# colinsongf/keyword_spotting

Hardware: AMD Instinct MI355X
Metric: mel-frames/s (real-time 10 ms-hop audio streams sustained = value/100) (higher is better)
Workload: dtype f32

## Files before the change

keyword_spotting_amd/csrc/gru_kernels.hip:

```cpp
#include <cstddef>

#include "gru_device.h"
#include "window_device.h"

namespace kws {

template <int KCX, bool FIRST, bool LAST, bool WINDOW = false>
__global__ void __launch_bounds__(256) __attribute__((amdgpu_waves_per_eu(1, 1)))
gru_layer_resident(const GruLayerParams p) {
    static_assert(!WINDOW || (LAST && !FIRST), "the window tail belongs to the last layer of a stack");
    constexpr int H = 128, NT = 8, KCH = 32;
    const int tid = threadIdx.x;
    const int w = __builtin_amdgcn_readfirstlane(tid >> 6);
    const int lane = tid & 63, g = lane >> 4, s = lane & 15;
    const int n_groups = (p.B + kStreamsPerGroup - 1) / kStreamsPerGroup;
    int group = blockIdx.x;
    int b_raw = group * kStreamsPerGroup + s;
    bool bvalid = b_raw < p.B;
    int b = bvalid ? b_raw : p.B - 1;
    const int T = p.T;
    const int n0 = 2 * w, n1 = 2 * w + 1;

    extern __shared__ __attribute__((aligned(16))) char smem[];
    f32x4* hbuf = reinterpret_cast<f32x4*>(smem);
    f32x4* rhbuf = hbuf + NT * 64;
    f32x4* wlds = rhbuf + NT * 64;
    EpilogueLds epi = epilogue_carve(reinterpret_cast<char*>(wlds + 4 * KCX * 64));
    if constexpr (WINDOW) epi.cwords = reinterpret_cast<int8_t*>(reinterpret_cast<char*>(wlds + 4 * KCX * 64) + kEpilogueLdsBytes);
    const uint8_t* win_dl = reinterpret_cast<const uint8_t*>(epi.cwords) + 16 * kWinTailWordsStride;
    constexpr size_t kWinOffset = offsetof(GruLayerParams, win);
    if constexpr (WINDOW) window_tail_prepare(window_tail_params_from_kernarg(kWinOffset), const_cast<uint8_t*>(win_dl), tid);
    constexpr int kXsStride = xs_stride(KCX);
    float* xs = reinterpret_cast<float*>(reinterpret_cast<char*>(wlds + 4 * KCX * 64) + (LAST ? kEpilogueLdsBytes : 0));

    float wgh[2][2][KCH];
    float wch[2][KCH];
    float wcx[2][KCX];
    const f32x4* wh4 = reinterpret_cast<const f32x4*>(p.wh);
#pragma unroll
    for (int j = 0; j < 2; ++j) {
        const int n = 2 * w + j;
#pragma unroll
        for (int k4 = 0; k4 < KCH / 4; ++k4) {
            const f32x4 vr = wh4[((n * 3 + 0) * (KCH / 4) + k4) * 64 + lane];
            const f32x4 vu = wh4[((n * 3 + 1) * (KCH / 4) + k4) * 64 + lane];
            const f32x4 vc = wh4[((n * 3 + 2) * (KCH / 4) + k4) * 64 + lane];
#pragma unroll
            for (int e = 0; e < 4; ++e) {
                wgh[j][0][4 * k4 + e] = vr[e];
                wgh[j][1][4 * k4 + e] = vu[e];
                wch[j][4 * k4 + e] = vc[e];
            }
        }
    }
    if constexpr (FIRST) {
#pragma unroll
        for (int j = 0; j < 2; ++j)
#pragma unroll
            for (int kc = 0; kc < KCX; ++kc) wcx[j][kc] = p.wx[(((2 * w + j) * 3 + 2) * KCX + kc) * 64 + lane];
        for (int kc = 0; kc < KCX; ++kc) {
            f32x4 v;
            v.x = p.wx[((n0 * 3 + 0) * KCX + kc) * 64 + lane];
            v.y = p.wx[((n0 * 3 + 1) * KCX + kc) * 64 + lane];
            v.z = p.wx[((n1 * 3 + 0) * KCX + kc) * 64 + lane];
            v.w = p.wx[((n1 * 3 + 1) * KCX + kc) * 64 + lane];
            wlds[(w * KCX + kc) * 64 + lane] = v;
        }
    } else {
        const f32x4* wx4 = reinterpret_cast<const f32x4*>(p.wx);
#pragma unroll
        for (int j = 0; j < 2; ++j)
#pragma unroll
            for (int k4 = 0; k4 < KCX / 4; ++k4) {
                const f32x4 vc = wx4[(((2 * w + j) * 3 + 2) * (KCX / 4) + k4) * 64 + lane];
#pragma unroll
                for (int e = 0; e < 4; ++e) wcx[j][4 * k4 + e] = vc[e];
            }
        for (int k4 = 0; k4 < KCX / 4; ++k4) {
            const f32x4 r0 = wx4[((n0 * 3 + 0) * (KCX / 4) + k4) * 64 + lane];
            const f32x4 u0 = wx4[((n0 * 3 + 1) * (KCX / 4) + k4) * 64 + lane];
            const f32x4 r1 = wx4[((n1 * 3 + 0) * (KCX / 4) + k4) * 64 + lane];
            const f32x4 u1 = wx4[((n1 * 3 + 1) * (KCX / 4) + k4) * 64 + lane];
#pragma unroll
            for (int e = 0; e < 4; ++e)
                wlds[(w * KCX + 4 * k4 + e) * 64 + lane] = (f32x4){r0[e], u0[e], r1[e], u1[e]};
        }
    }
#pragma unroll
    for (int j = 0; j < 2; ++j) {
#pragma unroll
        for (int kc = 0; kc < KCH; ++kc) {
            asm volatile("" : "+a"(wgh[j][0][kc]));
            asm volatile("" : "+a"(wgh[j][1][kc]));
            asm volatile("" : "+a"(wch[j][kc]));
        }
    }
    asm volatile("s_nop 7" ::: "memory");
    f32x4 bias_r[2], bias_u[2], bias_c[2];
#pragma unroll
    for (int j = 0; j < 2; ++j) {
        const int n = 2 * w + j;
        bias_r[j] = ld4(p.bias + 0 * H + n * 16 + 4 * g);
        bias_u[j] = ld4(p.bias + 1 * H + n * 16 + 4 * g);
        bias_c[j] = ld4(p.bias + 2 * H + n * 16 + 4 * g);
    }
    float wfc[2][4];
    f32x4 bfc4 = splat4(0.f);
    if (LAST) {
#pragma unroll
        for (int j = 0; j < 2; ++j)
#pragma unroll
            for (int e = 0; e < 4; ++e) wfc[j][e] = p.wfc[((2 * w + j) * 4 + e) * 64 + lane];
        if (w == 0) bfc4 = ld4(p.bfc + 4 * g);
    }

    int len_s = T;
    f32x4 hreg[2];
    const float4* xl_src = nullptr;
    const float4* xprev = nullptr;
    constexpr int XQ = KCX;
    const int xl_row = lane / XQ, xl_q = lane % XQ;
    const bool xl_active = FIRST && lane < 4 * XQ;
    auto enter_group = [&]() {
        b_raw = group * kStreamsPerGroup + s;
        bvalid = b_raw < p.B;
        b = bvalid ? b_raw : p.B - 1;
        const bool do_reset = p.reset != nullptr && p.reset[b] != 0;
        len_s = p.seq_len ? p.seq_len[b] - p.t_base : T;
#pragma unroll
        for (int j = 0; j < 2; ++j) {
            const int n = 2 * w + j;
            hreg[j] = do_reset ? splat4(0.f) : ld4(p.state_in + (size_t)b * H + n * 16 + 4 * g);
            hbuf[n * 64 + lane] = hreg[j];
        }
        if (LAST && tid < 16) {
            const int bb = group * kStreamsPerGroup + tid;
            int pw = -1;
            if (bb < p.B && p.prev_word && !(p.reset && p.reset[bb])) pw = p.prev_word[bb];
            epi.carry[tid] = pw;
        }
        if constexpr (FIRST) {
            const int xl_b = min(group * kStreamsPerGroup + 4 * w + (xl_active ? xl_row : 0), p.B - 1);
            xl_src = reinterpret_cast<const float4*>(p.x_mel + (size_t)xl_b * (p.t_stride ? p.t_stride : T) * p.I) + xl_q;
        } else {
            xprev = p.x_prev + (size_t)group * T * NT * 64 + lane;
        }
    };

    float4 xl_inflight = make_float4(0.f, 0.f, 0.f, 0.f);
    auto coop_issue = [&](int t_req) {
        const int t = t_req < T ? t_req : T - 1;
        if (xl_active) xl_inflight = xl_src[(size_t)t * XQ];
    };
    auto coop_commit = [&]() {
        if (xl_active) {
            float* dst = xs + (4 * (4 * w + xl_row)) * kXsStride + xl_q;
            dst[0 * kXsStride] = xl_inflight.x;
            dst[1 * kXsStride] = xl_inflight.y;
            dst[2 * kXsStride] = xl_inflight.z;
            dst[3 * kXsStride] = xl_inflight.w;
        }
    };
    float xbuf0[KCX];
    auto read_xs = [&](float (&dst)[KCX]) {
        const float* row = xs + (4 * s + g) * kXsStride;
#pragma unroll
        for (int k4 = 0; k4 < KCX / 4; ++k4) {
            const f32x4 v = *reinterpret_cast<const f32x4*>(row + 4 * k4);
            dst[4 * k4 + 0] = v[0]; dst[4 * k4 + 1] = v[1]; dst[4 * k4 + 2] = v[2]; dst[4 * k4 + 3] = v[3];
        }
        if constexpr (KCX % 4 >= 2) {
            const f32x2 v = *reinterpret_cast<const f32x2*>(row + (KCX / 4) * 4);
            dst[(KCX / 4) * 4 + 0] = v[0]; dst[(KCX / 4) * 4 + 1] = v[1];
        }
        if constexpr (KCX % 2 == 1) dst[KCX - 1] = row[KCX - 1];
    };
    auto load_x_slice = [&](float (&dst)[KCX], int t_req, const int sl) {
        if constexpr (!FIRST) {
            const int t = t_req < T ? t_req : T - 1;
            const float4 v = xprev[((size_t)t * NT + sl) * 64];
            dst[4 * sl + 0] = v.x; dst[4 * sl + 1] = v.y; dst[4 * sl + 2] = v.z; dst[4 * sl + 3] = v.w;
        }
    };

    f32x4 acc_r[2], acc_u[2], acc_c[2];
    auto gates_x_part = [&](const float (&xB)[KCX], auto k0_, auto k1_, auto pin_) {
        constexpr int K0 = decltype(k0_)::value, K1 = decltype(k1_)::value;
        constexpr bool PIN = decltype(pin_)::value;
        f32x4 ring[3];
        if (K0 < K1) ring[K0 % 3] = wlds[(w * KCX + K0) * 64 + lane];
        if (K0 + 1 < K1) ring[(K0 + 1) % 3] = wlds[(w * KCX + K0 + 1) * 64 + lane];
#pragma unroll
        for (int kc = K0; kc < K1; ++kc) {
            if (kc + 2 < K1) ring[(kc + 2) % 3] = wlds[(w * KCX + kc + 2) * 64 + lane];
            if (PIN) __builtin_amdgcn_sched_barrier(0);
            const f32x4 a4 = ring[kc % 3];
            acc_r[0] = mfma4(a4.x, xB[kc], acc_r[0]);
            acc_u[0] = mfma4(a4.y, xB[kc], acc_u[0]);
            acc_r[1] = mfma4(a4.z, xB[kc], acc_r[1]);
            acc_u[1] = mfma4(a4.w, xB[kc], acc_u[1]);
            if (PIN) __builtin_amdgcn_sched_barrier(0);
        }
    };
    using pinned = std::true_type;
    constexpr int KSPLIT = KCX / 2;
    using k_lo = std::integral_constant<int, 0>;
    using k_mid = std::integral_constant<int, KSPLIT>;
    using k_hi = std::integral_constant<int, KCX>;
    auto cand_x = [&](const float (&xB)[KCX]) {
#pragma unroll
        for (int j = 0; j < 2; ++j) acc_c[j] = bias_c[j];
#pragma unroll
        for (int kc = 0; kc < KCX; ++kc) {
            acc_c[0] = mfma4(wcx[0][kc], xB[kc], acc_c[0]);
            acc_c[1] = mfma4(wcx[1][kc], xB[kc], acc_c[1]);
        }
    };

    f32x4 hb_a, hb_b;

    auto frame = [&](int t, float (&xcur)[KCX], float (&xnxt)[KCX]) {
        mfma_prefence(acc_r[0], acc_u[0], acc_r[1], acc_u[1]);
#pragma unroll
        for (int nn = 0; nn < NT; ++nn) {
            const f32x4 hb = (nn & 1) ? hb_b : hb_a;
            if (nn + 2 < NT) {
                if (nn & 1) hb_b = hbuf[(nn + 2) * 64 + lane]; else hb_a = hbuf[(nn + 2) * 64 + lane];
            }
            if constexpr (FIRST) { if (nn == 0) coop_issue(t + 2); } else load_x_slice(xnxt, t + 1, nn);
            __builtin_amdgcn_sched_barrier(0);
#pragma unroll
            for (int e = 0; e < 4; ++e) {
                const int kc = 4 * nn + e;
                const float hv = hb[e];
                KWS_MFMA_A(acc_r[0], wgh[0][0][kc], hv);
                KWS_MFMA_A(acc_u[0], wgh[0][1][kc], hv);
                KWS_MFMA_A(acc_r[1], wgh[1][0][kc], hv);
                KWS_MFMA_A(acc_u[1], wgh[1][1][kc], hv);
            }
        }
        mfma_fence(acc_r[0], acc_u[0], acc_r[1], acc_u[1]);
        if constexpr (FIRST) read_xs(xcur);
        f32x4 u[2];
#pragma unroll
        for (int j = 0; j < 2; ++j) {
            const f32x2 r_lo = sigmoid2((f32x2){acc_r[j][0], acc_r[j][1]});
            const f32x2 r_hi = sigmoid2((f32x2){acc_r[j][2], acc_r[j][3]});
            const f32x2 rh_lo = r_lo * (f32x2){hreg[j][0], hreg[j][1]};
            const f32x2 rh_hi = r_hi * (f32x2){hreg[j][2], hreg[j][3]};
            rhbuf[(2 * w + j) * 64 + lane] = (f32x4){rh_lo.x, rh_lo.y, rh_hi.x, rh_hi.y};
        }
#pragma unroll
        for (int j = 0; j < 2; ++j) {
            const f32x2 u_lo = sigmoid2((f32x2){acc_u[j][0], acc_u[j][1]});
            const f32x2 u_hi = sigmoid2((f32x2){acc_u[j][2], acc_u[j][3]});
            u[j] = (f32x4){u_lo.x, u_lo.y, u_hi.x, u_hi.y};
        }
#pragma unroll
        for (int j = 0; j < 2; ++j) { acc_r[j] = bias_r[j]; acc_u[j] = bias_u[j]; }
        __builtin_amdgcn_sched_barrier(0);
        gates_x_part(xcur, k_lo{}, k_mid{}, pinned{});
        lds_barrier();
        hb_a = rhbuf[0 * 64 + lane];
        hb_b = rhbuf[1 * 64 + lane];
        gates_x_part(xcur, k_mid{}, k_hi{}, pinned{});

        mfma_prefence(acc_c[0], acc_c[1]);
#pragma unroll
        for (int nn = 0; nn < NT; ++nn) {
            const f32x4 rb = (nn & 1) ? hb_b : hb_a;
            if (nn + 2 < NT) {
                if (nn & 1) hb_b = rhbuf[(nn + 2) * 64 + lane]; else hb_a = rhbuf[(nn + 2) * 64 + lane];
            }
            __builtin_amdgcn_sched_barrier(0);
#pragma unroll
            for (int e = 0; e < 4; ++e) {
                const int kc = 4 * nn + e;
                const float rv = rb[e];
                KWS_MFMA_A(acc_c[0], wch[0][kc], rv);
                KWS_MFMA_A(acc_c[1], wch[1][kc], rv);
            }
        }
        mfma_fence(acc_c[0], acc_c[1]);
        const unsigned live = t < len_s ? 0xffffffffu : 0u;
        f32x4 hout[2];
#pragma unroll
        for (int j = 0; j < 2; ++j) {
#pragma unroll
            for (int h2 = 0; h2 < 2; ++h2) {
                const f32x2 c = tanh2((f32x2){acc_c[j][2 * h2], acc_c[j][2 * h2 + 1]});
                const f32x2 uu = {u[j][2 * h2], u[j][2 * h2 + 1]};
                const f32x2 hh = {hreg[j][2 * h2], hreg[j][2 * h2 + 1]};
                const f32x2 hn = (1.0f - uu) * c + uu * hh;
                hreg[j][2 * h2] = bitsel(live, hn.x, hh.x);
                hreg[j][2 * h2 + 1] = bitsel(live, hn.y, hh.y);
                if (LAST) {
                    hout[j][2 * h2] = bitsel(live, hn.x, 0.f);
                    hout[j][2 * h2 + 1] = bitsel(live, hn.y, 0.f);
                }
            }
        }
#pragma unroll
        for (int j = 0; j < 2; ++j) acc_c[j] = bias_c[j];
        constexpr int NCX = 2 * KCX;
        constexpr int NPOST = NCX >= 32 ? 16 : 8;
        constexpr int NPRE = NCX - NPOST;
        auto cand_x_mfma = [&](auto mc) {
            constexpr int m = decltype(mc)::value, kc = m / 2;
            if constexpr (m % 2 == 0) acc_c[0] = mfma4(wcx[0][kc], xcur[kc], acc_c[0]);
            else acc_c[1] = mfma4(wcx[1][kc], xcur[kc], acc_c[1]);
        };
        if constexpr (FIRST) coop_commit();
#pragma unroll
        for (int j = 0; j < 2; ++j) {
            hbuf[(2 * w + j) * 64 + lane] = hreg[j];
            if (!LAST) {
                const f32x4 o = hreg[j];
                p.h_out[((size_t)group * T + t) * NT * 64 + (2 * w + j) * 64 + lane] =
                    make_float4(o[0], o[1], o[2], o[3]);
            }
        }
        if (LAST) {
            f32x4 accf = bfc4;
#pragma unroll
            for (int j = 0; j < 2; ++j)
#pragma unroll
                for (int e = 0; e < 4; ++e) accf = mfma4(wfc[j][e], hout[j][e], accf);
            if (g < 2) *reinterpret_cast<f32x4*>(epi.pstage + (w * 16 + s) * 8 + 4 * g) = accf;
        }
        __builtin_amdgcn_sched_barrier(0);
        static_for<0, NPRE>(cand_x_mfma);
        __builtin_amdgcn_sched_barrier(0);
        lds_barrier();
        hb_a = hbuf[0 * 64 + lane];
        hb_b = hbuf[1 * 64 + lane];
        FoldRegs fold;
        const bool folder = LAST && w == (t & 3);
        if (folder) epilogue_fold_load(epi, lane, fold);
        __builtin_amdgcn_sched_barrier(0);
        static_for<NPRE, NCX>(cand_x_mfma);
        __builtin_amdgcn_sched_barrier(0);
        if (LAST) {
            if (folder) epilogue_fold_store(epi, t, lane, fold);
            if (((t + 1) & (kRingFrames - 1)) == 0 || t == T - 1) {
                const int t0 = t & ~(kRingFrames - 1);
                lds_barrier();
                epilogue_flush(p, epi, group, t0, t - t0 + 1, w, lane, t == T - 1);
            }
        }
    };

    for (; group < n_groups; group += gridDim.x) {
    enter_group();
    __syncthreads();
    if (T > 0) {
        if constexpr (FIRST) {
            coop_issue(0);
            coop_commit();
            __syncthreads();
            read_xs(xbuf0);
            coop_issue(1);
        } else {
#pragma unroll
            for (int sl = 0; sl < NT; ++sl) load_x_slice(xbuf0, 0, sl);
        }
#pragma unroll
        for (int j = 0; j < 2; ++j) { acc_r[j] = bias_r[j]; acc_u[j] = bias_u[j]; }
        gates_x_part(xbuf0, k_lo{}, k_hi{}, pinned{});
        hb_a = hbuf[0 * 64 + lane];
        hb_b = hbuf[1 * 64 + lane];
        cand_x(xbuf0);
        if constexpr (FIRST) {
            __syncthreads();
            coop_commit();
            __syncthreads();
        }
    }
    for (int t = 0; t < T; ++t) frame(t, xbuf0, xbuf0);

    if (bvalid) {
#pragma unroll
        for (int j = 0; j < 2; ++j)
            *reinterpret_cast<f32x4*>(p.state_out + (size_t)b * H + (2 * w + j) * 16 + 4 * g) = hreg[j];
    }
    __syncthreads();
    if constexpr (WINDOW) {
        const WindowTail win = window_tail_params_from_kernarg(kWinOffset);
        WindowTailRegs<2> wreq;
        window_tail_request<2>(win, p.B, group * kStreamsPerGroup, tid, wreq);
        window_tail<2>(win, p.B, group * kStreamsPerGroup, T, epi.cwords, kWinTailWordsStride, win_dl, reinterpret_cast<char*>(hbuf), tid, wreq);
        __syncthreads();
    }
    }
}

constexpr float kResidualScale = 0.7071067811865475f;
constexpr float kLayerNormEps = 1e-5f;

template <int TPW, bool FIRST, bool LAST, bool PIPE, bool WRAP = false>
__device__ __forceinline__ void gru_layer_generic_body(const GruLayerParams& p, const int group,
                                                       const GruWrapLayer& wl = GruWrapLayer{nullptr, 0.f, 0}) {
    constexpr int NT = 4 * TPW, H = 64 * TPW;
    const int tid = threadIdx.x;
    const int w = __builtin_amdgcn_readfirstlane(tid >> 6);
    const int lane = tid & 63, g = lane >> 4, s = lane & 15;
    const int b_raw = group * kStreamsPerGroup + s;
    const bool bvalid = b_raw < p.B;
    const int b = bvalid ? b_raw : p.B - 1;
    const int T = p.T, I = p.I;
    const int KCX4 = p.KCX / 4;

    extern __shared__ __attribute__((aligned(16))) char smem[];
    f32x4* hbuf = reinterpret_cast<f32x4*>(smem);
    f32x4* rhbuf = hbuf + NT * 64;
    f32x4* xstage = rhbuf + NT * 64;
    f32x4* biasl = xstage + NT * 64;
    const EpilogueLds epi = epilogue_carve(reinterpret_cast<char*>(biasl + 3 * NT * 4));
    f32x4* const xln = WRAP ? reinterpret_cast<f32x4*>(reinterpret_cast<char*>(biasl + 3 * NT * 4) + kEpilogueLdsBytes) : nullptr;
    const bool w_ln = WRAP && wl.igamma != nullptr;
    const bool w_res = WRAP && !FIRST && wl.residual != 0;
    const bool w_staged = w_ln || w_res;

    const __amdgpu_buffer_rsrc_t wx_rsrc = __builtin_amdgcn_make_buffer_rsrc(const_cast<float*>(p.wx), (short)0, 0x7fffffff, 0x00020000);
    const __amdgpu_buffer_rsrc_t wh_rsrc = __builtin_amdgcn_make_buffer_rsrc(const_cast<float*>(p.wh), (short)0, 0x7fffffff, 0x00020000);
    const int lane16 = lane * 16;
    auto bload = [&](const __amdgpu_buffer_rsrc_t& r, int frag) -> f32x4 {
        return __builtin_bit_cast(f32x4, __builtin_amdgcn_raw_buffer_load_b128(r, lane16, frag * 1024, 0));
    };

    f32x4 hreg[TPW];
    const bool do_reset = p.reset != nullptr && p.reset[b] != 0;
    const int len_s = p.seq_len ? p.seq_len[b] - p.t_base : T;
    for (int i = tid; i < 3 * NT * 4; i += 256) biasl[i] = ld4(p.bias + 4 * i);
#pragma unroll
    for (int j = 0; j < TPW; ++j) {
        const int n = TPW * w + j;
        hreg[j] = do_reset ? splat4(0.f) : ld4(p.state_in + (size_t)b * H + n * 16 + 4 * g);
        hbuf[n * 64 + lane] = hreg[j];
    }
    f32x4 bfc4 = splat4(0.f);
    if (LAST) {
        if (w == 0) bfc4 = ld4(p.bfc + 4 * g);
        if (tid < 16) {
            const int bb = group * kStreamsPerGroup + tid;
            int pw = -1;
            if (bb < p.B && p.prev_word && !(p.reset && p.reset[bb])) pw = p.prev_word[bb];
            epi.carry[tid] = pw;
        }
    }
    const float* xrow = FIRST ? p.x_mel + (size_t)b * (p.t_stride ? p.t_stride : T) * I : nullptr;
    const __amdgpu_buffer_rsrc_t xp_rsrc = __builtin_amdgcn_make_buffer_rsrc(
        FIRST ? const_cast<float*>(p.wh) : const_cast<float*>(reinterpret_cast<const float*>(p.x_prev + (size_t)group * T * NT * 64)),
        (short)0, 0x7fffffff, 0x00020000);
    const __amdgpu_buffer_rsrc_t ho_rsrc = __builtin_amdgcn_make_buffer_rsrc(
        LAST ? const_cast<float*>(p.wh) : reinterpret_cast<float*>(p.h_out + (size_t)group * T * NT * 64), (short)0, 0x7fffffff, 0x00020000);
    constexpr int kSysScope = 1 | 16;
    const bool vec_ok = (I & 3) == 0;
    __syncthreads();

    auto x_operand = [&](int t, int k4) -> f32x4 {
        f32x4 xb;
        if (WRAP && w_staged) {
            xb = (w_ln ? xln : xstage)[k4 * 64 + lane];
        } else if (FIRST) {
            const int k = 16 * k4 + 4 * g;
            const float* src = xrow + (size_t)t * I + k;
            if (vec_ok && k + 3 < I) {
                xb = ld4(src);
            } else {
#pragma unroll
                for (int e = 0; e < 4; ++e) xb[e] = (k + e < I) ? src[e] : 0.f;
            }
        } else if (PIPE) {
            xb = xstage[k4 * 64 + lane];
        } else {
            xb = bload(xp_rsrc, t * NT + k4);
        }
        return xb;
    };
    constexpr int RT = TPW, NP = TPW / RT;
    struct RowX { f32x4 a[RT][3]; f32x4 xb; };
    struct RowH { f32x4 a[RT][2]; };
    struct RowC { f32x4 a[RT]; };
    auto load_x = [&](RowX& r, int t, int q) {
        const int qq = q < KCX4 * NP ? q : KCX4 * NP - 1, kk = qq / NP, part = qq - kk * NP;
#pragma unroll
        for (int j = 0; j < RT; ++j)
#pragma unroll
            for (int c = 0; c < 3; ++c) r.a[j][c] = bload(wx_rsrc, ((TPW * w + part * RT + j) * 3 + c) * KCX4 + kk);
        r.xb = x_operand(t, kk);
        __builtin_amdgcn_sched_barrier(0);
    };
    auto load_h = [&](RowH& r, int q) {
        const int qq = q < NT * NP ? q : NT * NP - 1, kk = qq / NP, part = qq - kk * NP;
#pragma unroll
        for (int j = 0; j < RT; ++j)
#pragma unroll
            for (int c = 0; c < 2; ++c) r.a[j][c] = bload(wh_rsrc, ((TPW * w + part * RT + j) * 3 + c) * NT + kk);
        __builtin_amdgcn_sched_barrier(0);
    };
    auto load_c = [&](RowC& r, int q) {
        const int qq = q < NT * NP ? q : NT * NP - 1, kk = qq / NP, part = qq - kk * NP;
#pragma unroll
        for (int j = 0; j < RT; ++j) r.a[j] = bload(wh_rsrc, ((TPW * w + part * RT + j) * 3 + 2) * NT + kk);
        __builtin_amdgcn_sched_barrier(0);
    };
    auto mel_operand = [&](int t, int k4) -> f32x4 {
        f32x4 xb;
        const int k = 16 * k4 + 4 * g;
        const float* src = xrow + (size_t)t * I + k;
        if (vec_ok && k + 3 < I) {
            xb = ld4(src);
        } else {
#pragma unroll
            for (int e = 0; e < 4; ++e) xb[e] = (k + e < I) ? src[e] : 0.f;
        }
        return xb;
    };
    auto wrap_frame = [&](int t) {
        f32x4* const raw = FIRST ? xln : xstage;
        if (FIRST) {
            for (int k0 = w; k0 < KCX4; k0 += 16) {
                f32x4 v[4];
#pragma unroll
                for (int i = 0; i < 4; ++i) if (k0 + 4 * i < KCX4) v[i] = mel_operand(t, k0 + 4 * i);
#pragma unroll
                for (int i = 0; i < 4; ++i) if (k0 + 4 * i < KCX4) raw[(k0 + 4 * i) * 64 + lane] = v[i];
            }
            __syncthreads();
        } else if (!PIPE) {
            f32x4 v[NT / 4];
#pragma unroll
            for (int i = 0; i < NT / 4; ++i) v[i] = bload(xp_rsrc, t * NT + w + 4 * i);
#pragma unroll
            for (int i = 0; i < NT / 4; ++i) raw[(w + 4 * i) * 64 + lane] = v[i];
            __syncthreads();
        }
        if (!w_ln) return;
        float sum = 0.f;
        for (int k4 = 0; k4 < KCX4; ++k4) {
            const f32x4 v = raw[k4 * 64 + lane];
            sum += (v[0] + v[1]) + (v[2] + v[3]);
        }
        sum += __shfl_xor(sum, 16);
        sum += __shfl_xor(sum, 32);
        const float mu = sum / (float)I;
        float sq = 0.f;
        for (int k4 = 0; k4 < KCX4; ++k4) {
            const f32x4 v = raw[k4 * 64 + lane];
#pragma unroll
            for (int e = 0; e < 4; ++e) {
                float d = v[e] - mu;
                if (FIRST) d = (16 * k4 + 4 * g + e < I) ? d : 0.f;
                sq = fmaf(d, d, sq);
            }
        }
        sq += __shfl_xor(sq, 16);
        sq += __shfl_xor(sq, 32);
        const float scale = wl.ibeta * rsqrtf(sq / (float)I + kLayerNormEps);
        if (FIRST) __syncthreads();
        for (int k0 = w; k0 < KCX4; k0 += 16) {
            f32x4 gm[4];
#pragma unroll
            for (int i = 0; i < 4; ++i) if (k0 + 4 * i < KCX4) gm[i] = ld4(wl.igamma + 16 * (k0 + 4 * i) + 4 * g);
#pragma unroll
            for (int i = 0; i < 4; ++i) {
                const int k4 = k0 + 4 * i;
                if (k4 < KCX4) {
                    const f32x4 v = raw[k4 * 64 + lane];
                    f32x4 o;
#pragma unroll
                    for (int e = 0; e < 4; ++e) {
                        o[e] = fmaf(v[e] - mu, scale, gm[i][e]);
                        if (FIRST) o[e] = (16 * k4 + 4 * g + e < I) ? o[e] : 0.f;
                    }
                    xln[k4 * 64 + lane] = o;
                }
            }
        }
        __syncthreads();
    };
    for (int t = 0; t < T; ++t) {
        f32x4 acc_r[TPW], acc_u[TPW], acc_c[TPW];
#pragma unroll
        for (int j = 0; j < TPW; ++j) {
            const int n = TPW * w + j;
            acc_r[j] = biasl[(0 * NT + n) * 4 + g]; acc_u[j] = biasl[(1 * NT + n) * 4 + g]; acc_c[j] = biasl[(2 * NT + n) * 4 + g];
        }
        if (PIPE && !FIRST) {
            int spins = 0;
            while (__hip_atomic_load(p.ready_in + group, __ATOMIC_RELAXED, __HIP_MEMORY_SCOPE_AGENT) <= t) {
                __builtin_amdgcn_s_sleep(2);
                if (++spins > (1 << 24)) { if (lane == 0) *reinterpret_cast<volatile int*>(p.pipe_error) = 1; break; }
            }
            asm volatile("" ::: "memory");
            f32x4 xv[NT / 4];
#pragma unroll
            for (int i = 0; i < NT / 4; ++i)
                xv[i] = __builtin_bit_cast(f32x4, __builtin_amdgcn_raw_buffer_load_b128(xp_rsrc, lane16, (t * NT + (w + 4 * i)) * 1024, kSysScope));
#pragma unroll
            for (int i = 0; i < NT / 4; ++i) xstage[(w + 4 * i) * 64 + lane] = xv[i];
            __syncthreads();
        }
        if constexpr (WRAP) {
            if (w_staged) wrap_frame(t);
        }
        {
#define KWS_MMA_X(P_)                                                                                 \
            _Pragma("unroll") for (int j = 0; j < RT; ++j)                                             \
                _Pragma("unroll") for (int e = 0; e < 4; ++e) {                                        \
                    acc_r[P_ * RT + j] = mfma4(rr.a[j][0][e], rr.xb[e], acc_r[P_ * RT + j]);           \
                    acc_u[P_ * RT + j] = mfma4(rr.a[j][1][e], rr.xb[e], acc_u[P_ * RT + j]);           \
                    acc_c[P_ * RT + j] = mfma4(rr.a[j][2][e], rr.xb[e], acc_c[P_ * RT + j]);           \
                }
            RowX ra, rb;
            const int NQ = KCX4 * NP;
            load_x(ra, t, 0);
#pragma nounroll
            for (int q = 0; q < NQ; q += 2) {
                load_x(rb, t, q + 1);
                { const RowX& rr = ra; KWS_MMA_X(0); __builtin_amdgcn_sched_barrier(0); }
                if (q + 1 < NQ) {
                    load_x(ra, t, q + 2);
                    { const RowX& rr = rb; if (NP == 2) { KWS_MMA_X((NP - 1)); } else { KWS_MMA_X(0); } __builtin_amdgcn_sched_barrier(0); }
                }
            }
#undef KWS_MMA_X
        }
        {
#define KWS_MMA_H(P_)                                                                                 \
            _Pragma("unroll") for (int j = 0; j < RT; ++j)                                             \
                _Pragma("unroll") for (int e = 0; e < 4; ++e) {                                        \
                    acc_r[P_ * RT + j] = mfma4(rr.a[j][0][e], hb[e], acc_r[P_ * RT + j]);              \
                    acc_u[P_ * RT + j] = mfma4(rr.a[j][1][e], hb[e], acc_u[P_ * RT + j]);              \
                }
            RowH ra, rb;
            constexpr int NQ = NT * NP;
            load_h(ra, 0);
#pragma nounroll
            for (int q = 0; q < NQ; q += 2) {
                load_h(rb, q + 1);
                { const RowH& rr = ra; const f32x4 hb = hbuf[(q / NP) * 64 + lane]; KWS_MMA_H(0); __builtin_amdgcn_sched_barrier(0); }
                load_h(ra, q + 2);
                { const RowH& rr = rb; const f32x4 hb = hbuf[((q + 1) / NP) * 64 + lane];
                  if (NP == 2) { KWS_MMA_H((NP - 1)); } else { KWS_MMA_H(0); } __builtin_amdgcn_sched_barrier(0); }
            }
#undef KWS_MMA_H
        }
        f32x4 u[TPW];
#pragma unroll
        for (int j = 0; j < TPW; ++j) {
            f32x4 rh;
#pragma unroll
            for (int e = 0; e < 4; ++e) {
                rh[e] = sigmoid_f(acc_r[j][e]) * hreg[j][e];
                u[j][e] = sigmoid_f(acc_u[j][e]);
            }
            rhbuf[(TPW * w + j) * 64 + lane] = rh;
        }
        RowC ca, cb;
        if (PIPE && !LAST) asm volatile("s_waitcnt vmcnt(0)" ::: "memory");
        load_c(ca, 0);
        __syncthreads();
        if (PIPE && !LAST && t > 0 && tid == 0)
            __hip_atomic_store(p.ready_out + group, t, __ATOMIC_RELAXED, __HIP_MEMORY_SCOPE_AGENT);
        {
#define KWS_MMA_C(P_)                                                                                 \
            _Pragma("unroll") for (int j = 0; j < RT; ++j)                                             \
                _Pragma("unroll") for (int e = 0; e < 4; ++e)                                          \
                    acc_c[P_ * RT + j] = mfma4(rr.a[j][e], rb[e], acc_c[P_ * RT + j]);
            constexpr int NQ = NT * NP;
#pragma nounroll
            for (int q = 0; q < NQ; q += 2) {
                load_c(cb, q + 1);
                { const RowC& rr = ca; const f32x4 rb = rhbuf[(q / NP) * 64 + lane]; KWS_MMA_C(0); __builtin_amdgcn_sched_barrier(0); }
                load_c(ca, q + 2);
                { const RowC& rr = cb; const f32x4 rb = rhbuf[((q + 1) / NP) * 64 + lane];
                  if (NP == 2) { KWS_MMA_C((NP - 1)); } else { KWS_MMA_C(0); } __builtin_amdgcn_sched_barrier(0); }
            }
#undef KWS_MMA_C
        }
        const unsigned live = t < len_s ? 0xffffffffu : 0u;
        f32x4 accf = bfc4;
#pragma unroll
        for (int j = 0; j < TPW; ++j) {
            const int n = TPW * w + j;
            f32x4 hout;
            f32x4 xr = splat4(0.f), seam = splat4(0.f);
            if (WRAP && w_res) xr = xstage[n * 64 + lane];
#pragma unroll
            for (int e = 0; e < 4; ++e) {
                const float c = tanh_f(acc_c[j][e]);
                const float hn = fmaf(u[j][e], hreg[j][e], (1.0f - u[j][e]) * c);
                hreg[j][e] = bitsel(live, hn, hreg[j][e]);
                hout[e] = bitsel(live, hn, 0.f);
                if (WRAP) {
                    const float o = w_res ? kResidualScale * (hn + xr[e]) : hn;
                    hout[e] = bitsel(live, o, 0.f);
                    seam[e] = bitsel(live, o, hreg[j][e]);
                }
            }
            hbuf[n * 64 + lane] = hreg[j];
            if (!LAST) {
                const f32x4 o = WRAP ? seam : hreg[j];
                float4* dst = p.h_out + ((size_t)group * T + t) * NT * 64 + n * 64 + lane;
                if (PIPE) {
                    typedef int i32x4 __attribute__((ext_vector_type(4)));
                    __builtin_amdgcn_raw_buffer_store_b128(__builtin_bit_cast(i32x4, o), ho_rsrc, lane16, (t * NT + n) * 1024, kSysScope);
                } else {
                    *dst = make_float4(o[0], o[1], o[2], o[3]);
                }
            } else {
#pragma unroll
                for (int e = 0; e < 4; ++e) accf = mfma4(p.wfc[(n * 4 + e) * 64 + lane], hout[e], accf);
            }
        }
        if (LAST && g < 2) *reinterpret_cast<f32x4*>(epi.pstage + (w * 16 + s) * 8 + 4 * g) = accf;
        __syncthreads();
        if (LAST) {
            if (w == (t & 3)) epilogue_fold(epi, t, lane);
            if (((t + 1) & (kRingFrames - 1)) == 0 || t == T - 1) {
                const int t0 = t & ~(kRingFrames - 1);
                __syncthreads();
                epilogue_flush(p, epi, group, t0, t - t0 + 1, w, lane, t == T - 1);
            }
        }
    }
    if (PIPE && !LAST) {
        asm volatile("s_waitcnt vmcnt(0)" ::: "memory");
        __syncthreads();
        if (tid == 0) __hip_atomic_store(p.ready_out + group, T, __ATOMIC_RELAXED, __HIP_MEMORY_SCOPE_AGENT);
    }
    if (bvalid) {
#pragma unroll
        for (int j = 0; j < TPW; ++j)
            *reinterpret_cast<f32x4*>(p.state_out + (size_t)b * H + (TPW * w + j) * 16 + 4 * g) = hreg[j];
    }
}

template <int TPW, bool FIRST, bool LAST>
__global__ void __launch_bounds__(256) gru_layer_generic(const GruLayerParams p) {
    gru_layer_generic_body<TPW, FIRST, LAST, false>(p, blockIdx.x);
}

template <int TPW>
__global__ void __launch_bounds__(256) gru_stack_generic_pipelined(const GruStackParams sp) {
    int layer, group;
    if (sp.xcd_affine) {
        const int xcd = blockIdx.x & 7, slot = blockIdx.x >> 3, per = 8 / sp.L;
        layer = xcd % sp.L;
        group = slot * per + xcd / sp.L;
        if (group >= sp.G) return;
    } else {
        layer = blockIdx.x / sp.G;
        group = blockIdx.x - layer * sp.G;
    }
    if (layer == 0) gru_layer_generic_body<TPW, true, false, true>(sp.layer[0], group);
    else if (layer == sp.L - 1) gru_layer_generic_body<TPW, false, true, true>(sp.layer[layer], group);
    else gru_layer_generic_body<TPW, false, false, true>(sp.layer[layer], group);
}

template <int TPW, bool FIRST, bool LAST>
__global__ void __launch_bounds__(256) gru_layer_generic_wrapped(const GruLayerParams p, const GruWrapLayer wl) {
    gru_layer_generic_body<TPW, FIRST, LAST, false, true>(p, blockIdx.x, wl);
}
template <int TPW>
__global__ void __launch_bounds__(256) gru_stack_generic_pipelined_wrapped(const GruStackParams sp, const GruWrapParams wp) {
    int layer, group;
    if (sp.xcd_affine) {
        const int xcd = blockIdx.x & 7, slot = blockIdx.x >> 3, per = 8 / sp.L;
        layer = xcd % sp.L;
        group = slot * per + xcd / sp.L;
        if (group >= sp.G) return;
    } else {
        layer = blockIdx.x / sp.G;
        group = blockIdx.x - layer * sp.G;
    }
    if (layer == 0) gru_layer_generic_body<TPW, true, false, true, true>(sp.layer[0], group, wp.layer[0]);
    else if (layer == sp.L - 1) gru_layer_generic_body<TPW, false, true, true, true>(sp.layer[layer], group, wp.layer[layer]);
    else gru_layer_generic_body<TPW, false, false, true, true>(sp.layer[layer], group, wp.layer[layer]);
}
static_assert(sizeof(GruStackParams) + sizeof(GruWrapParams) <= 4096, "kernel arguments");

static size_t resident_lds_bytes(int kcx, bool first, bool last) {
    size_t n = 2 * 8 * 64 * 16 + (size_t)4 * kcx * 64 * 16;
    if (last) n += kEpilogueLdsBytes;
    if (first) n += (size_t)64 * xs_stride(kcx) * 4;
    return n;
}
constexpr size_t kOneWorkgroupPerCuLds = 82 * 1024;

static size_t generic_lds_bytes(int hidden, bool last) {
    size_t n = (size_t)3 * (hidden / 16) * 64 * 16 + (size_t)3 * hidden * 4;
    if (last) n += kEpilogueLdsBytes;
    return n;
}

int gru_resident_kcx(int in_dim, bool first) { return first ? (in_dim + 3) / 4 : 32; }

bool gru_resident_supported(int hidden, int in_dim, bool first) {
    if (hidden != 128) return false;
    if (!first) return in_dim == 128;
    return in_dim == 32 || in_dim == 40 || in_dim == 48 || in_dim == 60 || in_dim == 64;
}

template <typename K>
static hipError_t launch_with_lds(K kernel, const GruLayerParams& p, size_t lds, hipStream_t st) {
    static LdsGrant granted;
    {
        const hipError_t e = grant_dynamic_lds(kernel, granted, lds);
        if (e != hipSuccess) return e;
    }
    const int groups = (p.B + kStreamsPerGroup - 1) / kStreamsPerGroup;
    hipLaunchKernelGGL(kernel, dim3(groups), dim3(256), lds, st, p);
    return hipGetLastError();
}

static int device_cu_count() {
    static std::atomic<int> cached[kMaxDevices];
    int dev = 0;
    if (hipGetDevice(&dev) != hipSuccess || dev < 0 || dev >= kMaxDevices) return 256;
    int n = cached[dev].load(std::memory_order_relaxed);
    if (n <= 0) {
        hipDeviceProp_t prop;
        n = hipGetDeviceProperties(&prop, dev) == hipSuccess && prop.multiProcessorCount > 0 ? prop.multiProcessorCount : 256;
        cached[dev].store(n, std::memory_order_relaxed);
    }
    return n;
}
template <typename K>
static hipError_t launch_resident(K kernel, const GruLayerParams& p, size_t lds, hipStream_t st) {
    static LdsGrant granted;
    {
        const hipError_t e = grant_dynamic_lds(kernel, granted, lds);
        if (e != hipSuccess) return e;
    }
    const int groups = (p.B + kStreamsPerGroup - 1) / kStreamsPerGroup, cus = device_cu_count();
    hipLaunchKernelGGL(kernel, dim3(groups < cus ? groups : cus), dim3(256), lds, st, p);
    return hipGetLastError();
}

bool gru_resident_takes_window(bool first, bool last) { return last && !first; }

hipError_t launch_gru_layer_resident(const GruLayerParams& p, bool first, bool last, hipStream_t st) {
    const size_t lds = resident_lds_bytes(p.KCX, first, last);
    if (p.win.tab != nullptr) {
        if (!gru_resident_takes_window(first, last) || p.seq_len) return hipErrorInvalidValue;
        return launch_resident(gru_layer_resident<32, false, true, true>, p, lds + kWinTailWordsBytes, st);
    }
#define KWS_RES(KCX_, F_, L_) return launch_resident(gru_layer_resident<KCX_, F_, L_>, p, lds, st)
    if (first) {
        if (p.KCX == 8) { if (last) KWS_RES(8, true, true); else KWS_RES(8, true, false); }
        if (p.KCX == 10) { if (last) KWS_RES(10, true, true); else KWS_RES(10, true, false); }
        if (p.KCX == 12) { if (last) KWS_RES(12, true, true); else KWS_RES(12, true, false); }
        if (p.KCX == 15) { if (last) KWS_RES(15, true, true); else KWS_RES(15, true, false); }
        if (p.KCX == 16) { if (last) KWS_RES(16, true, true); else KWS_RES(16, true, false); }
        return hipErrorInvalidValue;
    }
    if (last) KWS_RES(32, false, true); else KWS_RES(32, false, false);
#undef KWS_RES
}

template <int TPW>
static hipError_t launch_pipelined(const GruStackParams& sp, size_t lds, hipStream_t st) {
    static LdsGrant granted;
    {
        const hipError_t e = grant_dynamic_lds(gru_stack_generic_pipelined<TPW>, granted, lds);
        if (e != hipSuccess) return e;
    }
    const int per = sp.xcd_affine ? 8 / sp.L : 0;
    const int grid = sp.xcd_affine ? 8 * ((sp.G + per - 1) / per) : sp.G * sp.L;
    hipLaunchKernelGGL(gru_stack_generic_pipelined<TPW>, dim3(grid), dim3(256), lds, st, sp);
    return hipGetLastError();
}

hipError_t launch_gru_stack_generic_pipelined(const GruStackParams& sp, int hidden, hipStream_t st) {
    size_t lds = generic_lds_bytes(hidden, true);
    if (lds < kOneWorkgroupPerCuLds) lds = kOneWorkgroupPerCuLds;
    if (hidden == 64) return launch_pipelined<1>(sp, lds, st);
    if (hidden == 128) return launch_pipelined<2>(sp, lds, st);
    if (hidden == 256) return launch_pipelined<4>(sp, lds, st);
    return hipErrorInvalidValue;
}

hipError_t launch_gru_layer_generic(const GruLayerParams& p, int hidden, bool first, bool last,
                                    hipStream_t st) {
    size_t lds = generic_lds_bytes(hidden, last);
    if (p.t_stride != 0 && lds < kOneWorkgroupPerCuLds) lds = kOneWorkgroupPerCuLds;
#define KWS_GEN(TPW_) \
    do { \
        if (first && last) return launch_with_lds(gru_layer_generic<TPW_, true, true>, p, lds, st); \
        if (first) return launch_with_lds(gru_layer_generic<TPW_, true, false>, p, lds, st); \
        if (last) return launch_with_lds(gru_layer_generic<TPW_, false, true>, p, lds, st); \
        return launch_with_lds(gru_layer_generic<TPW_, false, false>, p, lds, st); \
    } while (0)
    if (hidden == 64) KWS_GEN(1);
    if (hidden == 128) KWS_GEN(2);
    if (hidden == 256) KWS_GEN(4);
#undef KWS_GEN
    return hipErrorInvalidValue;
}

template <typename K>
static hipError_t launch_wrapped_with_lds(K kernel, const GruLayerParams& p, const GruWrapLayer& wl, size_t lds, hipStream_t st) {
    static LdsGrant granted;
    {
        const hipError_t e = grant_dynamic_lds(kernel, granted, lds);
        if (e != hipSuccess) return e;
    }
    const int groups = (p.B + kStreamsPerGroup - 1) / kStreamsPerGroup;
    hipLaunchKernelGGL(kernel, dim3(groups), dim3(256), lds, st, p, wl);
    return hipGetLastError();
}

hipError_t launch_gru_layer_generic_wrapped(const GruLayerParams& p, const GruWrapLayer& wl, int hidden, bool first, bool last,
                                            hipStream_t st) {
    size_t lds = generic_lds_bytes(hidden, true) + gru_wrapped_extra_lds(p.KCX / 4);
    if (p.t_stride != 0 && lds < kOneWorkgroupPerCuLds) lds = kOneWorkgroupPerCuLds;
#define KWS_GENW(TPW_) \
    do { \
        if (first && last) return launch_wrapped_with_lds(gru_layer_generic_wrapped<TPW_, true, true>, p, wl, lds, st); \
        if (first) return launch_wrapped_with_lds(gru_layer_generic_wrapped<TPW_, true, false>, p, wl, lds, st); \
        if (last) return launch_wrapped_with_lds(gru_layer_generic_wrapped<TPW_, false, true>, p, wl, lds, st); \
        return launch_wrapped_with_lds(gru_layer_generic_wrapped<TPW_, false, false>, p, wl, lds, st); \
    } while (0)
    if (hidden == 64) KWS_GENW(1);
    if (hidden == 128) KWS_GENW(2);
    if (hidden == 256) KWS_GENW(4);
#undef KWS_GENW
    return hipErrorInvalidValue;
}

template <int TPW>
static hipError_t launch_pipelined_wrapped(const GruStackParams& sp, const GruWrapParams& wp, size_t lds, hipStream_t st) {
    static LdsGrant granted;
    {
        const hipError_t e = grant_dynamic_lds(gru_stack_generic_pipelined_wrapped<TPW>, granted, lds);
        if (e != hipSuccess) return e;
    }
    const int per = sp.xcd_affine ? 8 / sp.L : 0;
    const int grid = sp.xcd_affine ? 8 * ((sp.G + per - 1) / per) : sp.G * sp.L;
    hipLaunchKernelGGL(gru_stack_generic_pipelined_wrapped<TPW>, dim3(grid), dim3(256), lds, st, sp, wp);
    return hipGetLastError();
}

hipError_t launch_gru_stack_generic_pipelined_wrapped(const GruStackParams& sp, const GruWrapParams& wp, int hidden, hipStream_t st) {
    int kx4 = 0;
    for (int l = 0; l < sp.L; ++l) kx4 = sp.layer[l].KCX / 4 > kx4 ? sp.layer[l].KCX / 4 : kx4;
    size_t lds = generic_lds_bytes(hidden, true) + gru_wrapped_extra_lds(kx4);
    if (lds < kOneWorkgroupPerCuLds) lds = kOneWorkgroupPerCuLds;
    if (hidden == 64) return launch_pipelined_wrapped<1>(sp, wp, lds, st);
    if (hidden == 128) return launch_pipelined_wrapped<2>(sp, wp, lds, st);
    if (hidden == 256) return launch_pipelined_wrapped<4>(sp, wp, lds, st);
    return hipErrorInvalidValue;
}

}
```

Measured before the change: 392.8 million.

## Stage next-frame GRU inputs through LDS and keep one input-weight chunk in registers

For non-first, non-window resident GRU layers, the previous layer's output for frame t+2 is now fetched cooperatively. Each wave issues two global loads per frame into registers, commits them to a new LDS staging buffer at frame end, and each lane reads its slices from LDS. This replaces per-slice global loads of frame t+1 inside the inner loop, aiming to hide global latency behind a full frame. It also moves the last input-weight chunk from LDS into registers to offset the added staging LDS and trim LDS reads. The cost is more register pressure, an extra LDS write/read per frame, and changed LDS sizing logic.

After: 394.7 million, median of 6. About the same (+0.5%).

```diff
diff --git a/keyword_spotting_amd/csrc/gru_kernels.hip b/keyword_spotting_amd/csrc/gru_kernels.hip
--- a/keyword_spotting_amd/csrc/gru_kernels.hip
+++ b/keyword_spotting_amd/csrc/gru_kernels.hip
@@ -4,6 +4,8 @@
 #include "window_device.h"
 
 namespace kws {
+
+constexpr int resident_kreg(bool first, bool window) { return !first && !window ? 1 : 0; }
 
 template <int KCX, bool FIRST, bool LAST, bool WINDOW = false>
 __global__ void __launch_bounds__(256) __attribute__((amdgpu_waves_per_eu(1, 1)))
@@ -21,21 +23,26 @@
     const int T = p.T;
     const int n0 = 2 * w, n1 = 2 * w + 1;
 
+    constexpr bool XSTAGE = !FIRST && !WINDOW;
+    constexpr int KREG = resident_kreg(FIRST, WINDOW), KL = KCX - KREG;
     extern __shared__ __attribute__((aligned(16))) char smem[];
     f32x4* hbuf = reinterpret_cast<f32x4*>(smem);
     f32x4* rhbuf = hbuf + NT * 64;
     f32x4* wlds = rhbuf + NT * 64;
-    EpilogueLds epi = epilogue_carve(reinterpret_cast<char*>(wlds + 4 * KCX * 64));
-    if constexpr (WINDOW) epi.cwords = reinterpret_cast<int8_t*>(reinterpret_cast<char*>(wlds + 4 * KCX * 64) + kEpilogueLdsBytes);
+    f32x4* xstage = wlds + 4 * KL * 64;
+    char* const lds_tail = reinterpret_cast<char*>(xstage + (XSTAGE ? NT * 64 : 0));
+    EpilogueLds epi = epilogue_carve(lds_tail);
+    if constexpr (WINDOW) epi.cwords = reinterpret_cast<int8_t*>(lds_tail + kEpilogueLdsBytes);
     const uint8_t* win_dl = reinterpret_cast<const uint8_t*>(epi.cwords) + 16 * kWinTailWordsStride;
     constexpr size_t kWinOffset = offsetof(GruLayerParams, win);
     if constexpr (WINDOW) window_tail_prepare(window_tail_params_from_kernarg(kWinOffset), const_cast<uint8_t*>(win_dl), tid);
     constexpr int kXsStride = xs_stride(KCX);
-    float* xs = reinterpret_cast<float*>(reinterpret_cast<char*>(wlds + 4 * KCX * 64) + (LAST ? kEpilogueLdsBytes : 0));
+    float* xs = reinterpret_cast<float*>(lds_tail + (LAST ? kEpilogueLdsBytes : 0));
 
     float wgh[2][2][KCH];
     float wch[2][KCH];
     float wcx[2][KCX];
+    f32x4 wxreg[KREG > 0 ? KREG : 1];
     const f32x4* wh4 = reinterpret_cast<const f32x4*>(p.wh);
 #pragma unroll
     for (int j = 0; j < 2; ++j) {
@@ -64,7 +71,7 @@
             v.y = p.wx[((n0 * 3 + 1) * KCX + kc) * 64 + lane];
             v.z = p.wx[((n1 * 3 + 0) * KCX + kc) * 64 + lane];
             v.w = p.wx[((n1 * 3 + 1) * KCX + kc) * 64 + lane];
-            wlds[(w * KCX + kc) * 64 + lane] = v;
+            wlds[(w * KL + kc) * 64 + lane] = v;
         }
     } else {
         const f32x4* wx4 = reinterpret_cast<const f32x4*>(p.wx);
@@ -83,7 +90,20 @@
             const f32x4 u1 = wx4[((n1 * 3 + 1) * (KCX / 4) + k4) * 64 + lane];
 #pragma unroll
             for (int e = 0; e < 4; ++e)
-                wlds[(w * KCX + 4 * k4 + e) * 64 + lane] = (f32x4){r0[e], u0[e], r1[e], u1[e]};
+                if (4 * k4 + e < KL) wlds[(w * KL + 4 * k4 + e) * 64 + lane] = (f32x4){r0[e], u0[e], r1[e], u1[e]};
+        }
+        if constexpr (KREG > 0) {
+            static_assert(KREG <= 4, "the register chunks come from the last group of four");
+            constexpr int k4 = KCX / 4 - 1;
+            const f32x4 r0 = wx4[((n0 * 3 + 0) * (KCX / 4) + k4) * 64 + lane];
+            const f32x4 u0 = wx4[((n0 * 3 + 1) * (KCX / 4) + k4) * 64 + lane];
+            const f32x4 r1 = wx4[((n1 * 3 + 0) * (KCX / 4) + k4) * 64 + lane];
+            const f32x4 u1 = wx4[((n1 * 3 + 1) * (KCX / 4) + k4) * 64 + lane];
+#pragma unroll
+            for (int i = 0; i < KREG; ++i) {
+                const int e = 4 - KREG + i;
+                wxreg[i] = (f32x4){r0[e], u0[e], r1[e], u1[e]};
+            }
         }
     }
 #pragma unroll
@@ -183,18 +203,34 @@
         }
     };
 
+    float4 xg_inflight[2] = {make_float4(0.f, 0.f, 0.f, 0.f), make_float4(0.f, 0.f, 0.f, 0.f)};
+    auto stage_issue = [&](int t_req, const int j) {
+        const int t = t_req < T ? t_req : T - 1;
+        xg_inflight[j] = xprev[((size_t)t * NT + 2 * w + j) * 64];
+    };
+    auto stage_commit = [&]() {
+#pragma unroll
+        for (int j = 0; j < 2; ++j)
+            xstage[(2 * w + j) * 64 + lane] = (f32x4){xg_inflight[j].x, xg_inflight[j].y, xg_inflight[j].z, xg_inflight[j].w};
+    };
+    auto read_stage_slice = [&](float (&dst)[KCX], const int sl) {
+        const f32x4 v = xstage[sl * 64 + lane];
+        dst[4 * sl + 0] = v[0]; dst[4 * sl + 1] = v[1]; dst[4 * sl + 2] = v[2]; dst[4 * sl + 3] = v[3];
+    };
+
     f32x4 acc_r[2], acc_u[2], acc_c[2];
     auto gates_x_part = [&](const float (&xB)[KCX], auto k0_, auto k1_, auto pin_) {
         constexpr int K0 = decltype(k0_)::value, K1 = decltype(k1_)::value;
         constexpr bool PIN = decltype(pin_)::value;
         f32x4 ring[3];
-        if (K0 < K1) ring[K0 % 3] = wlds[(w * KCX + K0) * 64 + lane];
-        if (K0 + 1 < K1) ring[(K0 + 1) % 3] = wlds[(w * KCX + K0 + 1) * 64 + lane];
+        constexpr int KE = K1 < KL ? K1 : KL;
+        if (K0 < KE) ring[K0 % 3] = wlds[(w * KL + K0) * 64 + lane];
+        if (K0 + 1 < KE) ring[(K0 + 1) % 3] = wlds[(w * KL + K0 + 1) * 64 + lane];
 #pragma unroll
         for (int kc = K0; kc < K1; ++kc) {
-            if (kc + 2 < K1) ring[(kc + 2) % 3] = wlds[(w * KCX + kc + 2) * 64 + lane];
+            if (kc + 2 < KE) ring[(kc + 2) % 3] = wlds[(w * KL + kc + 2) * 64 + lane];
             if (PIN) __builtin_amdgcn_sched_barrier(0);
-            const f32x4 a4 = ring[kc % 3];
+            const f32x4 a4 = kc < KL ? ring[kc % 3] : wxreg[kc < KL ? 0 : kc - KL];
             acc_r[0] = mfma4(a4.x, xB[kc], acc_r[0]);
             acc_u[0] = mfma4(a4.y, xB[kc], acc_u[0]);
             acc_r[1] = mfma4(a4.z, xB[kc], acc_r[1]);
@@ -227,7 +263,15 @@
             if (nn + 2 < NT) {
                 if (nn & 1) hb_b = hbuf[(nn + 2) * 64 + lane]; else hb_a = hbuf[(nn + 2) * 64 + lane];
             }
-            if constexpr (FIRST) { if (nn == 0) coop_issue(t + 2); } else load_x_slice(xnxt, t + 1, nn);
+            if constexpr (FIRST) {
+                if (nn == 0) coop_issue(t + 2);
+            } else if constexpr (XSTAGE) {
+                read_stage_slice(xnxt, nn);
+                if (nn == 0) stage_issue(t + 2, 0);
+                if (nn == NT / 2) stage_issue(t + 2, 1);
+            } else {
+                load_x_slice(xnxt, t + 1, nn);
+            }
             __builtin_amdgcn_sched_barrier(0);
 #pragma unroll
             for (int e = 0; e < 4; ++e) {
@@ -311,6 +355,7 @@
             else acc_c[1] = mfma4(wcx[1][kc], xcur[kc], acc_c[1]);
         };
         if constexpr (FIRST) coop_commit();
+        if constexpr (XSTAGE) stage_commit();
 #pragma unroll
         for (int j = 0; j < 2; ++j) {
             hbuf[(2 * w + j) * 64 + lane] = hreg[j];
@@ -360,6 +405,13 @@
             __syncthreads();
             read_xs(xbuf0);
             coop_issue(1);
+        } else if constexpr (XSTAGE) {
+            stage_issue(0, 0); stage_issue(0, 1);
+            stage_commit();
+            __syncthreads();
+#pragma unroll
+            for (int sl = 0; sl < NT; ++sl) read_stage_slice(xbuf0, sl);
+            stage_issue(1, 0); stage_issue(1, 1);
         } else {
 #pragma unroll
             for (int sl = 0; sl < NT; ++sl) load_x_slice(xbuf0, 0, sl);
@@ -370,9 +422,9 @@
         hb_a = hbuf[0 * 64 + lane];
         hb_b = hbuf[1 * 64 + lane];
         cand_x(xbuf0);
-        if constexpr (FIRST) {
+        if constexpr (FIRST || XSTAGE) {
             __syncthreads();
-            coop_commit();
+            if constexpr (FIRST) coop_commit(); else stage_commit();
             __syncthreads();
         }
     }
@@ -782,8 +834,9 @@
 }
 static_assert(sizeof(GruStackParams) + sizeof(GruWrapParams) <= 4096, "kernel arguments");
 
-static size_t resident_lds_bytes(int kcx, bool first, bool last) {
-    size_t n = 2 * 8 * 64 * 16 + (size_t)4 * kcx * 64 * 16;
+static size_t resident_lds_bytes(int kcx, bool first, bool last, bool window) {
+    size_t n = 2 * 8 * 64 * 16 + (size_t)4 * (kcx - resident_kreg(first, window)) * 64 * 16;
+    if (!first && !window) n += 8 * 64 * 16;
     if (last) n += kEpilogueLdsBytes;
     if (first) n += (size_t)64 * xs_stride(kcx) * 4;
     return n;
@@ -843,7 +896,7 @@
 bool gru_resident_takes_window(bool first, bool last) { return last && !first; }
 
 hipError_t launch_gru_layer_resident(const GruLayerParams& p, bool first, bool last, hipStream_t st) {
-    const size_t lds = resident_lds_bytes(p.KCX, first, last);
+    const size_t lds = resident_lds_bytes(p.KCX, first, last, p.win.tab != nullptr);
     if (p.win.tab != nullptr) {
         if (!gru_resident_takes_window(first, last) || p.seq_len) return hipErrorInvalidValue;
         return launch_resident(gru_layer_resident<32, false, true, true>, p, lds + kWinTailWordsBytes, st);
```
